# adamwalker/sdr

Hardware: AMD Instinct MI355X
Metric: Msamples/s through FM pipeline (decim8->demod->resamp3/10->filt) (higher is better)
Workload: dtype f32; 1 GPU; full FM chain (u8 IQ -> decim8 127 taps -> fmDemod -> resamp 3/10 191 taps -> 128-tap sym filter -> *0.2), 8192-sample block seams; blocks_per_gpu_per_pass=65536, samples_per_gpu_per_pass=536870912, passes_per_exchange=1, devices_visible=1, order=AVX (bit-exact vs reference AVX path)

## Files before the change

### sdr_amd/csrc/kernels_systolic.hip

```cpp
#include <atomic>
#include <stdlib.h>
#include <type_traits>
#include <utility>

#include "kernels.hpp"
#include "first_mac.hpp"
#include "decimate_tile.hpp"

namespace sdrhip {
namespace {

typedef float f2 __attribute__((ext_vector_type(2)));
typedef float f8 __attribute__((ext_vector_type(8)));

template <int PT>
struct Sys {
    static_assert(PT == 16 || PT == 8, "tap rows: a multiple of four (output 0 of a group then completes one stage before the others)");
    static constexpr int kWarm = (PT + 2) / 4;
    static constexpr int kOuts = 4 * (64 - kWarm);
    static constexpr int kStep = 8 * kOuts;
    static constexpr int kM = PT + 3;
};
constexpr int kStripOuts = Sys<16>::kOuts;
constexpr int kStripSpan = 2048;
constexpr int kWavesPerWg = 4;

__device__ __forceinline__ float dpp_shr1(float v)
{
    return __builtin_bit_cast(float, __builtin_amdgcn_update_dpp(0, __builtin_bit_cast(int, v), 0x138, 0xf, 0xf, true));
}

template <int... Ms, class F>
__device__ __forceinline__ void for_each_m(std::integer_sequence<int, Ms...>, F&& f)
{
    (f(std::integral_constant<int, Ms>{}), ...);
}

__device__ __forceinline__ f8 load_tap_row(const float* taps, int b)
{
    typedef const __attribute__((address_space(4))) f8* ctapp;
    uint64_t a = reinterpret_cast<uint64_t>(taps) + 32u * (uint32_t)b;
    asm volatile("" : "+s"(a));
    return *reinterpret_cast<ctapp>(a);
}

__device__ __forceinline__ void convert_u8x16(const uint4 raw, f2* S)
{
    const uint32_t w[4] = {raw.x ^ 0x80808080u, raw.y ^ 0x80808080u, raw.z ^ 0x80808080u, raw.w ^ 0x80808080u};
#pragma unroll
    for (int k = 0; k < 4; k++) {
        S[2 * k] = f2{(float)(signed char)(w[k] & 0xff), (float)(signed char)((w[k] >> 8) & 0xff)};
        S[2 * k + 1] = f2{(float)(signed char)((w[k] >> 16) & 0xff), (float)(signed char)(w[k] >> 24)};
    }
}

constexpr int kCfRow = 36;
constexpr int kCfWaveDw = 64 * kCfRow;

template <bool U8, bool WHOLE, bool NTL>
__device__ __forceinline__ void load_strip(const void* __restrict__ in, int64_t strip_s0, int64_t avail, float* __restrict__ wbuf, int lane, f2 (&S)[32])
{
    if constexpr (U8) {
        const uint8_t* base = reinterpret_cast<const uint8_t*>(in) + 2 * (strip_s0 + 32 * lane);
        uint4 raw[4];
        if constexpr (WHOLE) {
#pragma unroll
            for (int q = 0; q < 4; q++) raw[q] = reinterpret_cast<const uint4*>(base)[q];
        } else {
#pragma unroll
            for (int q = 0; q < 4; q++) {
                const int64_t s = 32 * lane + 8 * q;
                if (s + 8 <= avail) {
                    raw[q] = reinterpret_cast<const uint4*>(base)[q];
                } else {
                    uint32_t w[4] = {0x80808080u, 0x80808080u, 0x80808080u, 0x80808080u};
                    for (int e = 0; e < 16; e++)
                        if (s + e / 2 < avail) w[e >> 2] = (w[e >> 2] & ~(0xffu << (8 * (e & 3)))) | ((uint32_t)base[16 * q + e] << (8 * (e & 3)));
                    raw[q] = make_uint4(w[0], w[1], w[2], w[3]);
                }
            }
        }
#pragma unroll
        for (int q = 0; q < 4; q++) convert_u8x16(raw[q], &S[8 * q]);
    } else {
        const float* base = reinterpret_cast<const float*>(in) + 2 * strip_s0;
#pragma unroll
        for (int h = 0; h < 2; h++) {
            float4 v[8];
#pragma unroll
            for (int j = 0; j < 8; j++) {
                const int row = 8 * j + (lane >> 3);
                const int s = 32 * row + 16 * h + 2 * (lane & 7);
                const float* p = base + 2 * s;
                if (WHOLE || s + 2 <= avail) {
                    typedef float f4v __attribute__((ext_vector_type(4)));
                    if constexpr (NTL) {
                        const f4v t4 = __builtin_nontemporal_load(reinterpret_cast<const f4v*>(p));
                        v[j] = make_float4(t4.x, t4.y, t4.z, t4.w);
                    } else {
                        v[j] = *reinterpret_cast<const float4*>(p);
                    }
                } else {
                    v[j] = make_float4(0.f, 0.f, 0.f, 0.f);
                    if (s < avail) { v[j].x = p[0]; v[j].y = p[1]; }
                }
            }
#pragma unroll
            for (int j = 0; j < 8; j++) *reinterpret_cast<float4*>(wbuf + kCfRow * (8 * j + (lane >> 3)) + 4 * (lane & 7)) = v[j];
#pragma unroll
            for (int q = 0; q < 8; q++) {
                const float4 t = *reinterpret_cast<const float4*>(wbuf + kCfRow * lane + 4 * q);
                S[16 * h + 2 * q] = f2{t.x, t.y};
                S[16 * h + 2 * q + 1] = f2{t.z, t.w};
            }
        }
    }
}

struct SystolicFix {
    Geom g;
    const float* xtaps;
    int64_t first_seam;
    int nseams;
    int nfix_groups;
    int period_g;
    int seamK;
    int k0mod;
    int nx;
    int lp;
};
constexpr int kFixPer = 16, kFixSpw = 16;
constexpr int kFixLdsFloats = 2 * kFixSpw * crossfix_row_float2<8, 128, kFixPer>();

template <bool U8, int PSKIP, bool WHOLE, bool NTL, bool FIX, int PT>
__device__ __forceinline__ void systolic_strip(const void* __restrict__ in, int64_t x0, int strip, int count, const float* __restrict__ taps,
                                               float* __restrict__ out, float* __restrict__ wbuf, int lane, const SystolicFix& fx)
{
    constexpr int kOuts = Sys<PT>::kOuts, kStep = Sys<PT>::kStep, kWarm = Sys<PT>::kWarm;
    const int seamK = fx.seamK, k0mod = fx.k0mod, nx = fx.nx;
    f2 S[32];
    const int64_t strip_s0 = x0 + (int64_t)kStep * strip;
    const int64_t avail = WHOLE ? kStripSpan : ((int64_t)(count - 1) * 8 + fx.lp) - (int64_t)kStep * strip;
    load_strip<U8, WHOLE, NTL>(in, strip_s0, avail, wbuf, lane, S);

    f2 acc[4][4];
    f8 tc[PT];
    tc[0] = load_tap_row(taps, 0);
    auto do_m = [&](auto mc) {
        constexpr int m = decltype(mc)::value, t = m >> 2, c = m & 3;
        if constexpr (m + 1 < PT) tc[m + 1] = load_tap_row(taps, m + 1);
        else asm volatile("" ::: "memory");
#pragma unroll
        for (int r = 0; r < 8; r++) {
            const int k = r & 3;
#pragma unroll
            for (int i = 0; i < 4; i++) {
                const int b = (m - i) & (PT - 1);
                if (m - i < 0 || m - i > PT - 1) continue;
                if (PSKIP && 8 * b + r >= 8 * PT - PSKIP) {
                    if (t > 0 && c == 0 && r < 4) acc[i][k] = f2{dpp_shr1(acc[i][k].x), dpp_shr1(acc[i][k].y)};
                    continue;
                }
                if (b == 0 && r < 4) {
                    acc[i][k] = first_mac(S[8 * c + r], tc[b][r]);
                    continue;
                }
                const f2 p = S[8 * c + r] * tc[b][r];
                if (t > 0 && c == 0 && r < 4) {
                    acc[i][k] = f2{dpp_shr1(acc[i][k].x) + p.x, dpp_shr1(acc[i][k].y) + p.y};
                } else {
                    acc[i][k] = acc[i][k] + p;
                }
            }
        }
    };
    for_each_m(std::make_integer_sequence<int, Sys<PT>::kM>{}, do_m);

#pragma unroll
    for (int i = 0; i < 4; i++)
#pragma unroll
        for (int k = 0; k < 4; k++) asm volatile("" : "+v"(acc[i][k]));
    f2 res[4];
#pragma unroll
    for (int i = 0; i < 4; i++) res[i] = (acc[i][0] + acc[i][1]) + (acc[i][2] + acc[i][3]);
    res[0] = f2{dpp_shr1(res[0].x), dpp_shr1(res[0].y)};
    int km_strip = 0;
    bool strip_cross = false;
    if constexpr (FIX) {
        const int su = __builtin_amdgcn_readfirstlane(strip);
        km_strip = (int)(((unsigned)k0mod + (unsigned)((kOuts * (int64_t)su) % seamK)) % (unsigned)seamK);
        strip_cross = km_strip + (kOuts - 1) >= seamK - nx;
    }
    if (lane >= kWarm) {
        const int o = kOuts * strip + 4 * (lane - kWarm);
        bool cross[4] = {false, false, false, false};
        bool any_cross = false;
        if constexpr (FIX) {
            if (strip_cross) {
#pragma unroll
                for (int i = 0; i < 4; i++) {
                    int km = km_strip + 4 * (lane - kWarm) + i;
                    if (km >= seamK) km -= seamK;
                    cross[i] = km >= seamK - nx;
                    any_cross |= cross[i];
                }
            }
        }
        if ((WHOLE || o + 4 <= count) && !any_cross) {
            float4* dst = reinterpret_cast<float4*>(out + 2 * (int64_t)o);
            dst[0] = make_float4(res[0].x, res[0].y, res[1].x, res[1].y);
            dst[1] = make_float4(res[2].x, res[2].y, res[3].x, res[3].y);
        } else {
#pragma unroll
            for (int i = 0; i < 4; i++)
                if ((WHOLE || o + i < count) && !cross[i]) *reinterpret_cast<float2*>(out + 2 * (int64_t)(o + i)) = make_float2(res[i].x, res[i].y);
        }
    }
}

template <bool U8, int PSKIP, bool NTL = true, bool FIX = false, int PT = 16>
__global__ void __launch_bounds__(64 * kWavesPerWg, 4) k_decimate_systolic(const void* __restrict__ in, int64_t x0 ,
                                                                          int count, const float* __restrict__ taps, float* __restrict__ out,
                                                                          int nwhole , int nstrips, SystolicFix fx)
{
    constexpr int kStripLds = U8 ? 4 : kWavesPerWg * kCfWaveDw;
    __shared__ __attribute__((aligned(16))) float tbuf[FIX && kFixLdsFloats > kStripLds ? kFixLdsFloats : kStripLds];
    const int lane = threadIdx.x & 63, wave = threadIdx.x >> 6;
    int b = blockIdx.x;
    if constexpr (FIX) {
        const int G = b >> 6, q = G / fx.period_g;
        if (q < fx.nfix_groups && G - q * fx.period_g == fx.period_g - 1) {
            decimate_c_crossfix_wg<U8, 8, (PT == 16 ? 128 : 52), kFixPer, kFixSpw>(reinterpret_cast<float2*>(tbuf), 64 * q + (b & 63), fx.g, fx.xtaps, in, out, fx.first_seam, fx.nseams);
            return;
        }
        b -= 64 * (q < fx.nfix_groups ? q : fx.nfix_groups);
    }
    const int wg = (b & ~63) + ((b & 7) << 3) + ((b >> 3) & 7);
    const int strip = wg * kWavesPerWg + wave;
    if (strip >= nstrips) return;
    float* wbuf = tbuf + (U8 ? 0 : kCfWaveDw * wave);
    if (strip < nwhole) systolic_strip<U8, PSKIP, true, NTL, FIX, PT>(in, x0, strip, count, taps, out, wbuf, lane, fx);
    else systolic_strip<U8, PSKIP, false, NTL, FIX, PT>(in, x0, strip, count, taps, out, wbuf, lane, fx);
}

std::atomic<int>& systolic_flag()
{
    static std::atomic<int> f{getenv("SDRHIP_SYSTOLIC") ? atoi(getenv("SDRHIP_SYSTOLIC")) : 2};
    return f;
}
std::atomic<long long> g_systolic_launches{0};
std::atomic<long long> g_systolic_plain_launches{0};

}

static void systolic_plan_for(int count, int outs, int lp, int* nstrips, int* nwhole)
{
    *nstrips = (count + outs - 1) / outs;
    int w = count / outs;
    while (w > 0 && (int64_t)8 * outs * (w - 1) + kStripSpan > (int64_t)(count - 1) * 8 + lp) w--;
    *nwhole = w;
}
void systolic_plan(int count, int* nstrips, int* nwhole) { systolic_plan_for(count, kStripOuts, 128, nstrips, nwhole); }

void set_systolic(int mode) { systolic_flag().store(mode); }
long long systolic_launch_count() { return g_systolic_launches.load(); }
long long systolic_plain_launch_count() { return g_systolic_plain_launches.load(); }

constexpr int64_t kPlainLoadMinOutputs = (int64_t)1000 * 1024;
constexpr int64_t kPlainLoadMaxOutputs = (int64_t)4400 * 1024;
constexpr int64_t kFixInsideMaxOutputs = (int64_t)1 << 23;

bool launch_decimate_c4_systolic(hipStream_t s, const Geom& g, const float* d_taps, int P, const void* d_in, bool in_is_u8, float* d_out,
                                 bool last_tap_zero, const float* d_cross_taps, bool* seams_done)
{
    if (seams_done) *seams_done = false;
    const int mode = systolic_flag().load(std::memory_order_relaxed);
    if (mode == 0) return false;
    const bool p52 = in_is_u8 && mode == 2 && P == 52 && g.Lp == 52;
    if (g.I != 1 || g.D != 8 || !((P == 128 && g.Lp == 128) || p52) || g.count < 64 * kStripOuts * kWavesPerWg) return false;
    const int64_t x0 = g.k_begin * g.D - g.in_base;
    const uintptr_t base = reinterpret_cast<uintptr_t>(d_in);
    if (((base + (in_is_u8 ? 2 : 8) * (uintptr_t)x0) & 15) != 0 || (reinterpret_cast<uintptr_t>(d_out) & 15) != 0) return false;
    int nstrips, nwhole;
    systolic_plan_for(g.count, p52 ? Sys<8>::kOuts : Sys<16>::kOuts, g.Lp, &nstrips, &nwhole);
    const int nwg = (nstrips + kWavesPerWg - 1) / kWavesPerWg;
    int groups = (nwg + 63) / 64;
    SystolicFix fx = {};
    fx.lp = g.Lp;
    fx.nx = (g.Lp - 1) / 8;
    bool fix = false;
    if (mode == 2 && g.count <= kFixInsideMaxOutputs && seams_done && g.seamBI > 0 && g.seamBI % 8 == 0 && g.seamBI / 8 >= 256 && g.seamBI / 8 < (1 << 30) && d_cross_taps != nullptr) {
        const SeamSpan sp = seam_span(g);
        if (sp.nseams > 0) {
            fx.g = g;
            fx.xtaps = d_cross_taps;
            fx.first_seam = sp.first;
            fx.nseams = sp.nseams;
            fx.nfix_groups = ((fx.nseams + kFixSpw - 1) / kFixSpw + 63) / 64;
            fx.period_g = (groups + fx.nfix_groups) / fx.nfix_groups;
            fx.seamK = (int)(g.seamBI / 8);
            fx.k0mod = (int)(g.k_begin % fx.seamK);
            fix = fx.period_g >= 2;
        } else {
            *seams_done = true;
        }
    }
    if (fix) {
        groups += fx.nfix_groups;
        *seams_done = true;
    }
    const dim3 grid(groups * 64), block(64 * kWavesPerWg);
    const bool plain = !in_is_u8 && mode == 2 && g.count >= kPlainLoadMinOutputs && g.count <= kPlainLoadMaxOutputs;
#define SYS(U8V, PSKIPV, NTLV)                                                                                                                      \
    do {                                                                                                                                            \
        if (fix) hipLaunchKernelGGL((k_decimate_systolic<U8V, PSKIPV, NTLV, true>), grid, block, 0, s, d_in, x0, g.count, d_taps, d_out, nwhole, nstrips, fx); \
        else hipLaunchKernelGGL((k_decimate_systolic<U8V, PSKIPV, NTLV, false>), grid, block, 0, s, d_in, x0, g.count, d_taps, d_out, nwhole, nstrips, fx); \
    } while (0)
    if (p52) {
        if (fix) hipLaunchKernelGGL((k_decimate_systolic<true, 12, true, true, 8>), grid, block, 0, s, d_in, x0, g.count, d_taps, d_out, nwhole, nstrips, fx);
        else hipLaunchKernelGGL((k_decimate_systolic<true, 12, true, false, 8>), grid, block, 0, s, d_in, x0, g.count, d_taps, d_out, nwhole, nstrips, fx);
    } else if (in_is_u8 && last_tap_zero) SYS(true, 1, true);
    else if (in_is_u8) SYS(true, 0, true);
    else if (plain) SYS(false, 0, false);
    else SYS(false, 0, true);
#undef SYS
    g_systolic_launches.fetch_add(1, std::memory_order_relaxed);
    if (plain) g_systolic_plain_launches.fetch_add(1, std::memory_order_relaxed);
    return true;
}

}
```

Measured before the change: 587,300 Msamples/s.

## Software-pipeline systolic MAC: batch products ahead of accumulations with sched barriers

Splits the fused multiply-add inner loop of the systolic strip into separate product and addition phases, double-buffering products so the next row group's multiplies are issued before the current group's DPP-shifted accumulations. The batch size adapts to how many diagonal rows are live at each stage. Sched barriers pin this ordering so the multiplies can hide DPP and dependency latency. In exchange it needs more registers for the product buffers and removes the compiler's freedom to reorder.

```diff
diff --git a/sdr_amd/csrc/kernels_systolic.hip b/sdr_amd/csrc/kernels_systolic.hip
--- a/sdr_amd/csrc/kernels_systolic.hip
+++ b/sdr_amd/csrc/kernels_systolic.hip
@@ -20,6 +20,11 @@
     static constexpr int kOuts = 4 * (64 - kWarm);
     static constexpr int kStep = 8 * kOuts;
     static constexpr int kM = PT + 3;
+    static constexpr int batch_rows(int m)
+    {
+        const int live = (m < 3 ? m : 3) - (m - (PT - 1) > 0 ? m - (PT - 1) : 0) + 1;
+        return live >= 3 ? 1 : (live == 2 ? 2 : 4);
+    }
 };
 constexpr int kStripOuts = Sys<16>::kOuts;
 constexpr int kStripSpan = 2048;
@@ -146,12 +151,26 @@
     f2 acc[4][4];
     f8 tc[PT];
     tc[0] = load_tap_row(taps, 0);
-    auto do_m = [&](auto mc) {
-        constexpr int m = decltype(mc)::value, t = m >> 2, c = m & 3;
-        if constexpr (m + 1 < PT) tc[m + 1] = load_tap_row(taps, m + 1);
-        else asm volatile("" ::: "memory");
-#pragma unroll
-        for (int r = 0; r < 8; r++) {
+    f2 p[2][4][4];
+    auto products = [&](auto mc, int rg, f2 (&pb)[4][4]) {
+        constexpr int m = decltype(mc)::value, c = m & 3, G = Sys<PT>::batch_rows(m);
+#pragma unroll
+        for (int r = rg; r < rg + G; r++) {
+#pragma unroll
+            for (int i = 0; i < 4; i++) {
+                const int b = (m - i) & (PT - 1);
+                if (m - i < 0 || m - i > PT - 1) continue;
+                if (PSKIP && 8 * b + r >= 8 * PT - PSKIP) continue;
+                if (b == 0 && r < 4) continue;
+                pb[r - rg][i] = S[8 * c + r] * tc[b][r];
+            }
+        }
+        __builtin_amdgcn_sched_barrier(0);
+    };
+    auto additions = [&](auto mc, int rg, const f2 (&pb)[4][4]) {
+        constexpr int m = decltype(mc)::value, t = m >> 2, c = m & 3, G = Sys<PT>::batch_rows(m);
+#pragma unroll
+        for (int r = rg; r < rg + G; r++) {
             const int k = r & 3;
 #pragma unroll
             for (int i = 0; i < 4; i++) {
@@ -165,13 +184,26 @@
                     acc[i][k] = first_mac(S[8 * c + r], tc[b][r]);
                     continue;
                 }
-                const f2 p = S[8 * c + r] * tc[b][r];
+                const f2 q = pb[r - rg][i];
                 if (t > 0 && c == 0 && r < 4) {
-                    acc[i][k] = f2{dpp_shr1(acc[i][k].x) + p.x, dpp_shr1(acc[i][k].y) + p.y};
+                    acc[i][k] = f2{dpp_shr1(acc[i][k].x) + q.x, dpp_shr1(acc[i][k].y) + q.y};
                 } else {
-                    acc[i][k] = acc[i][k] + p;
-                }
-            }
+                    acc[i][k] = acc[i][k] + q;
+                }
+            }
+        }
+        __builtin_amdgcn_sched_barrier(0);
+    };
+    auto do_m = [&](auto mc) {
+        constexpr int m = decltype(mc)::value, G = Sys<PT>::batch_rows(m);
+        if constexpr (m + 1 < PT) tc[m + 1] = load_tap_row(taps, m + 1);
+        else asm volatile("" ::: "memory");
+        if constexpr (m == 0) products(mc, 0, p[0]);
+#pragma unroll
+        for (int n = 0; n < 8 / G; n++) {
+            if (n + 1 < 8 / G) products(mc, G * (n + 1), p[(n + 1) & 1]);
+            else if constexpr (m + 1 < Sys<PT>::kM) products(std::integral_constant<int, m + 1>{}, 0, p[0]);
+            additions(mc, G * n, p[n & 1]);
         }
     };
     for_each_m(std::make_integer_sequence<int, Sys<PT>::kM>{}, do_m);
```

Measured after the change: 591,800 Msamples/s (median of 6 runs). No clear change (+0.8%).
